# MIT-SPARK/TEASER-plusplus

Hardware: AMD Instinct MI355X
Metric: registrations/sec at N=10000 correspondences, 95% outliers (higher is better)
Workload: dtype bf16x3-split MFMA + f32 filter with FP64 fix-up for K1 (bitmap bit-identical to FP64); f64 estimators

## Files before the change

### teaser-plusplus_amd/csrc/kernels_graph.hip

```cpp
#include <algorithm>
#include <utility>
#include <vector>

#include <cstdio>
#include <cstdlib>

#include "internal.h"
#include "fixup_item.h"
#include "fixup_regions.h"
#include "k1_consts.h"
#include "wave_utils.h"

namespace thip {

struct EdgeConst {
  double beta;
  double beta2;
  double m2beta2;
  double beta4;
  double s_hat;
};

__device__ __forceinline__ bool tim_edge_exact(double ax, double ay, double az, double bx,
                                               double by, double bz, double beta) {
  const double A = (ax * ax + ay * ay) + az * az;
  const double B = (bx * bx + by * by) + bz * bz;
  return __builtin_fabs(__builtin_sqrt(A) - __builtin_sqrt(B)) <= beta;
}

__device__ __forceinline__ bool tim_edge_fast(double ax, double ay, double az, double bx,
                                              double by, double bz, const EdgeConst& k,
                                              bool* uncertain, bool* short_pair) {
  const double A = __builtin_fma(az, az, __builtin_fma(ay, ay, ax * ax));
  const double B = __builtin_fma(bz, bz, __builtin_fma(by, by, bx * bx));
  const double t = A + B;
  const double D = A - B;
  const double d = __builtin_fma(D, D, __builtin_fma(t, k.m2beta2, k.beta4));
  const double band = __builtin_fma(t, t, k.beta4) * 2e-12;
  *uncertain = !(__builtin_fabs(d) > band);
  *short_pair = t <= k.beta2;
  return d <= 0.0;
}

__device__ __forceinline__ bool tim_edge_scaled(double ax, double ay, double az, double bx,
                                                double by, double bz, const EdgeConst& k) {
  const double v1 = __builtin_sqrt((ax * ax + ay * ay) + az * az);
  const double v2 = __builtin_sqrt((bx * bx + by * by) + bz * bz);
  const double raw = v2 / v1;
  const double alpha = k.beta * (1.0 / v1);
  return __builtin_fabs(raw - k.s_hat) <= alpha;
}

constexpr int kColTilesPerWave = 4;
constexpr int kWavesPerBlock = 4;
constexpr int kColTilesPerBlock = kColTilesPerWave * kWavesPerBlock;

typedef double d2 __attribute__((ext_vector_type(2)));

template <int MODE>
struct ColTile {
  static constexpr int kPf = 3;
  const double* cb;
  d2 pf[kPf][3];
  int cb_addr;

  template <int C>
  __device__ __forceinline__ void load_col(d2 (&slot)[3]) {
    asm volatile("ds_read_b128 %0, %1 offset:%2" : "=v"(slot[0]) : "v"(cb_addr), "n"(48 * C));
    asm volatile("ds_read_b128 %0, %1 offset:%2" : "=v"(slot[1]) : "v"(cb_addr), "n"(48 * C + 16));
    asm volatile("ds_read_b128 %0, %1 offset:%2" : "=v"(slot[2]) : "v"(cb_addr), "n"(48 * C + 32));
  }
  double six, siy, siz, dix, diy, diz;
  unsigned int own_lo, own_hi;
  int tr_lo, tr_hi;
  uint64_t unc_cols;

  template <int B>
  __device__ __forceinline__ void step(const EdgeConst& kc) {
    constexpr int S = B % kPf;
    constexpr int younger = 3 * ((63 - B) < (kPf - 1) ? (63 - B) : (kPf - 1));
    asm volatile("s_waitcnt lgkmcnt(%3)" : "+v"(pf[S][0]), "+v"(pf[S][1]), "+v"(pf[S][2]) : "n"(younger));
    const double sjx = pf[S][0].x, sjy = pf[S][0].y, sjz = pf[S][1].x;
    const double djx = pf[S][1].y, djy = pf[S][2].x, djz = pf[S][2].y;
    if (B + kPf < 64) load_col<B + kPf>(pf[S]);
    bool e;
    uint64_t m;
    if (MODE == 0) {
      bool unc, shortp;
      const bool neg = tim_edge_fast(sjx - six, sjy - siy, sjz - siz, djx - dix, djy - diy,
                                     djz - diz, kc, &unc, &shortp);
      unc_cols |= (__builtin_amdgcn_ballot_w64(unc) != 0ull) ? (1ull << B) : 0ull;
      m = __builtin_amdgcn_ballot_w64(neg) | __builtin_amdgcn_ballot_w64(shortp);
// ... 211 lines not shown
  double H = 0.0;
  for (int k = 0; k < 6; ++k) {
    const float hi = f32_unkey(pr->hi[k]), lo = f32_unkey(~pr->lo[k]);
    const double e = 0.5 * ((double)hi - (double)lo);
    H = e > H ? e : H;
  }
  return H;
}

__global__ __launch_bounds__(256) void tim_prep_pack2_kernel(const ProbDesc* __restrict__ descs,
                                                             const double* __restrict__ src,
                                                             const double* __restrict__ dst,
                                                             TimPrep* __restrict__ prep,
                                                             TimOperandTile2* __restrict__ ops,
                                                             int32_t* __restrict__ deg, double beta) {
  const ProbDesc d = descs[blockIdx.y];
  const int ip = blockIdx.x * 256 + threadIdx.x;
  float mx = 0.f;
  if (ip < d.W * 64 && d.n > 0) {
    double g;
    int kexp;
    k1c::scale(beta, &g, &kexp);
    const int i = min(ip, d.n - 1);
    const TimPrep* pr = prep + blockIdx.y;
    const int sh = k1c::norm_shift(prep_half_extent(pr));
    kexp += 2 * sh;
    g *= k1c::pow2_d(sh);
    const double* a = src + 3 * (d.pt_off + i);
    const double* b = dst + 3 * (d.pt_off + i);
    const float sx = (float)((a[0] - prep_centre(pr, 0, 0)) * g), sy = (float)((a[1] - prep_centre(pr, 0, 1)) * g),
                sz = (float)((a[2] - prep_centre(pr, 0, 2)) * g);
    const float dx = (float)((b[0] - prep_centre(pr, 1, 0)) * g), dy = (float)((b[1] - prep_centre(pr, 1, 1)) * g),
                dz = (float)((b[2] - prep_centre(pr, 1, 2)) * g);
    const double na_d = ((double)sx * sx + (double)sy * sy) + (double)sz * sz;
    const double nb_d = ((double)dx * dx + (double)dy * dy) + (double)dz * dz;
    const float na = (float)na_d, nb = (float)nb_d;
    int ra, rb, pa, pb;
    k1c::xy_shifts(kexp, &ra, &rb, &pa, &pb);
    const float fra = (float)k1c::pow2_d(-ra), frb = (float)k1c::pow2_d(-rb), fpa = (float)k1c::pow2_d(-pa);
    const unsigned short P = f16_bits((float)k1c::pow2_d(-pb));
    unsigned short A[32], B[32];
    for (int k = 0; k < 32; ++k) A[k] = B[k] = 0;
    const float cs[3] = {sx, sy, sz}, cd[3] = {dx, dy, dz};
    float h, m, l;
    for (int c = 0; c < 3; ++c) {
      f16_split3(cs[c] * fra, &h, &m, &l);
      A[3 * c] = f16_bits(h); A[3 * c + 1] = A[3 * c]; A[3 * c + 2] = f16_bits(m);
      f16_split3(cs[c] * frb, &h, &m, &l);
      B[3 * c] = f16_bits(2.0f * h); B[3 * c + 1] = f16_bits(2.0f * m); B[3 * c + 2] = B[3 * c];
      f16_split3(cd[c] * fra, &h, &m, &l);
      A[16 + 3 * c] = f16_bits(h); A[16 + 3 * c + 1] = A[16 + 3 * c]; A[16 + 3 * c + 2] = f16_bits(m);
      f16_split3(cd[c] * frb, &h, &m, &l);
      B[16 + 3 * c] = f16_bits(-2.0f * h); B[16 + 3 * c + 1] = f16_bits(-2.0f * m); B[16 + 3 * c + 2] = B[16 + 3 * c];
    }
    f16_split3(na * fpa, &h, &m, &l);
    A[9] = f16_bits(-h); A[10] = f16_bits(-m); A[11] = f16_bits(-l); B[9] = P; B[10] = P; B[11] = P;
    B[12] = A[9]; B[13] = A[10]; B[14] = A[11]; A[12] = P; A[13] = P; A[14] = P;
    f16_split3(nb * fpa, &h, &m, &l);
    A[25] = f16_bits(h); A[26] = f16_bits(m); A[27] = f16_bits(l); B[25] = P; B[26] = P; B[27] = P;
    B[28] = A[25]; B[29] = A[26]; B[30] = A[27]; A[28] = P; A[29] = P; A[30] = P;
    A[31] = 0xb400;
    B[31] = 0x3c00;
    TimOperandTile2* tile = ops + d.w_off + (ip >> 6);
    const int gq = (ip >> 5) & 1, cc = ip & 31;
    for (int mf = 0; mf < kTimRowOperands; ++mf)
      for (int hh = 0; hh < 2; ++hh) {
        const unsigned short* pa = A + 16 * mf + 8 * hh;
        tile->a[gq][mf][hh][cc] = make_uint4(pa[0] | ((unsigned int)pa[1] << 16), pa[2] | ((unsigned int)pa[3] << 16),
                                             pa[4] | ((unsigned int)pa[5] << 16), pa[6] | ((unsigned int)pa[7] << 16));
        if (mf >= kTimColOperands) continue;
        const unsigned short* pb = B + 16 * mf + 8 * hh;
        tile->b[gq][mf][hh][cc] = make_uint4(pb[0] | ((unsigned int)pb[1] << 16), pb[2] | ((unsigned int)pb[3] << 16),
                                             pb[4] | ((unsigned int)pb[5] << 16), pb[6] | ((unsigned int)pb[7] << 16));
      }
    mx = na > nb ? na : nb;
    if (!(mx == mx)) mx = INFINITY;
    if (ip < d.n) deg[d.pt_off + ip] = 0;
  }
  for (int o = 32; o > 0; o >>= 1) {
    const float t = __shfl_xor(mx, o, 64);
    mx = t > mx ? t : mx;
  }
  if ((threadIdx.x & 63) == 0 && mx > 0.f) atomicMax(&prep[blockIdx.y].r2_bits, __float_as_uint(mx));
}

#ifdef TEASER_K1_LAB
struct TimOperandTile3 {
  uint4 a[2][3][2][32];
  uint4 b[2][2][2][32];
};
__global__ __launch_bounds__(256) void tim_prep_pack3_kernel(const ProbDesc* __restrict__ descs,
                                                             const double* __restrict__ src,
                                                             const double* __restrict__ dst,
                                                             TimPrep* __restrict__ prep,
                                                             TimOperandTile3* __restrict__ ops,
                                                             int32_t* __restrict__ deg, double beta) {
  const ProbDesc d = descs[blockIdx.y];
  const int ip = blockIdx.x * 256 + threadIdx.x;
  float mx = 0.f;
  if (ip < d.W * 64 && d.n > 0) {
    double g;
    int kexp;
    k1c::scale(beta, &g, &kexp);
    const int i = min(ip, d.n - 1);
    const TimPrep* pr = prep + blockIdx.y;
    const int sh = k1c::norm_shift(prep_half_extent(pr));
    kexp += 2 * sh;
    g *= k1c::pow2_d(sh);
    const double* a = src + 3 * (d.pt_off + i);
    const double* b = dst + 3 * (d.pt_off + i);
    const float sx = (float)((a[0] - prep_centre(pr, 0, 0)) * g), sy = (float)((a[1] - prep_centre(pr, 0, 1)) * g),
                sz = (float)((a[2] - prep_centre(pr, 0, 2)) * g);
    const float dx = (float)((b[0] - prep_centre(pr, 1, 0)) * g), dy = (float)((b[1] - prep_centre(pr, 1, 1)) * g),
                dz = (float)((b[2] - prep_centre(pr, 1, 2)) * g);
    const double na_d = ((double)sx * sx + (double)sy * sy) + (double)sz * sz;
    const double nb_d = ((double)dx * dx + (double)dy * dy) + (double)dz * dz;
    const float na = (float)na_d, nb = (float)nb_d;
    const double beta2s = k1c::pow2_d(kexp - 2);
    const float kappa = (float)k1c::pow2_d(kexp);
    const float delta_row = (float)(nb_d - na_d - beta2s);
    const float delta_col = (float)(nb_d - na_d);
    unsigned short A[48], B[32];
    for (int k = 0; k < 48; ++k) A[k] = 0;
    for (int k = 0; k < 32; ++k) B[k] = 0;
    const float cs[3] = {sx, sy, sz}, cd[3] = {dx, dy, dz};
    const unsigned short one = 0x3c00;
    float h, m, l;
    for (int c = 0; c < 3; ++c) {
      f16_split3(cs[c], &h, &m, &l);
      B[3 * c] = f16_bits(2.0f * h); B[3 * c + 1] = f16_bits(2.0f * m); B[3 * c + 2] = B[3 * c];
      A[3 * c] = f16_bits(h); A[3 * c + 1] = A[3 * c]; A[3 * c + 2] = f16_bits(m);
      A[32 + 3 * c] = f16_bits(kappa * h); A[32 + 3 * c + 1] = A[32 + 3 * c]; A[32 + 3 * c + 2] = f16_bits(kappa * m);
      f16_split3(cd[c], &h, &m, &l);
      B[16 + 3 * c] = f16_bits(-2.0f * h); B[16 + 3 * c + 1] = f16_bits(-2.0f * m); B[16 + 3 * c + 2] = B[16 + 3 * c];
      A[16 + 3 * c] = f16_bits(h); A[16 + 3 * c + 1] = A[16 + 3 * c]; A[16 + 3 * c + 2] = f16_bits(m);
    }
    f16_split3(na, &h, &m, &l);
    B[9] = f16_bits(-h); B[10] = f16_bits(-m);
    A[32 + 9] = f16_bits(kappa); A[32 + 10] = A[32 + 9];
    B[11] = one; B[12] = one; B[13] = one;
    B[14] = f16_bits(kappa); B[15] = B[14];
    A[32 + 14] = f16_bits(-h); A[32 + 15] = f16_bits(-m);
    f16_split3(delta_row, &h, &m, &l);
    A[11] = f16_bits(h); A[12] = f16_bits(m); A[13] = f16_bits(l);
    f16_split3(delta_col, &h, &m, &l);
    A[25] = one; A[26] = one; A[27] = one; B[25] = f16_bits(h); B[26] = f16_bits(m); B[27] = f16_bits(l);
    TimOperandTile3* tile = ops + d.w_off + (ip >> 6);
    const int gq = (ip >> 5) & 1, cc = ip & 31;
    for (int mf = 0; mf < 3; ++mf)
      for (int hh = 0; hh < 2; ++hh) {
        const unsigned short* pa = A + 16 * mf + 8 * hh;
        tile->a[gq][mf][hh][cc] = make_uint4(pa[0] | ((unsigned int)pa[1] << 16), pa[2] | ((unsigned int)pa[3] << 16),
                                             pa[4] | ((unsigned int)pa[5] << 16), pa[6] | ((unsigned int)pa[7] << 16));
        if (mf >= kTimColOperands) continue;
        const unsigned short* pb = B + 16 * mf + 8 * hh;
        tile->b[gq][mf][hh][cc] = make_uint4(pb[0] | ((unsigned int)pb[1] << 16), pb[2] | ((unsigned int)pb[3] << 16),
                                             pb[4] | ((unsigned int)pb[5] << 16), pb[6] | ((unsigned int)pb[7] << 16));
      }
    mx = na > nb ? na : nb;
    if (!(mx == mx)) mx = INFINITY;
    if (ip < d.n) deg[d.pt_off + ip] = 0;
  }
  for (int o = 32; o > 0; o >>= 1) {
    const float t = __shfl_xor(mx, o, 64);
    mx = t > mx ? t : mx;
  }
  if ((threadIdx.x & 63) == 0 && mx > 0.f) atomicMax(&prep[blockIdx.y].r2_bits, __float_as_uint(mx));
}
#endif

__global__ void tim_prep_consts_kernel(TimPrep* __restrict__ prep, int batch, double beta) {
  const int p = blockIdx.x * blockDim.x + threadIdx.x;
  if (p >= batch) return;
  const k1c::ConstsXY c = k1c::consts_xy(beta, k1c::norm_shift(prep_half_extent(prep + p)), prep[p].r2_bits);
  prep[p].band_c = c.C;
  prep[p].use_mfma = c.use_mfma;
}
#ifdef TEASER_K1_LAB
__global__ void tim_prep_consts3_kernel(TimPrep* __restrict__ prep, int batch, double beta) {
  const int p = blockIdx.x * blockDim.x + threadIdx.x;
  if (p >= batch) return;
  const k1c::Consts c = k1c::consts(beta, k1c::norm_shift(prep_half_extent(prep + p)), prep[p].r2_bits);
  prep[p].band_c = c.C;
  prep[p].use_mfma = c.use_mfma;
}
#endif


constexpr bool kK1Pipe = false, kK1Plain = true;
constexpr int kK1Chunks = 1, kK1Occ = 3;

template <bool PIPE, bool PLAIN, int OCC, int CHUNKS, bool LOWER, bool UW3 = false>
__global__ __launch_bounds__(256, OCC) void tim_graph_mfma3_kernel(
    const ProbDesc* __restrict__ descs, const double* __restrict__ src,
    const double* __restrict__ dst, const void* __restrict__ ops, const TimPrep* __restrict__ prep,
    uint64_t* __restrict__ bitmap, double beta, int gyr,
    unsigned long long* __restrict__ work, unsigned int* __restrict__ work_count,
    ProbState* __restrict__ states, int32_t* __restrict__ deg, unsigned long long* __restrict__ regions, int Tmax) {
  const ProbDesc d = descs[blockIdx.y];
  const int n = d.n, W = d.W;
  const int T = W;
  int Ig, X;
  fxr::decode_block((int)blockIdx.x, (int)gridDim.x, gyr, CHUNKS, &Ig, &X);
  constexpr int kBlockColTiles = kMfmaColTiles * CHUNKS;
  const int I0 = Ig * kMfmaRowTiles, Jbase = X * kBlockColTiles;
  auto region_of = [&](int wv, int chunk) -> unsigned long long* {
    const int Iw = I0 + wv, Xc = X * CHUNKS + chunk;
    return fxr::is_cell(Iw, Xc, Tmax) ? regions + fxr::region_offset((int)blockIdx.y, Tmax, Iw, Xc) : nullptr;
  };
  auto zero_regions = [&]() {
    if ((threadIdx.x & 63) < CHUNKS) {
      unsigned long long* r = region_of((int)(threadIdx.x >> 6), (int)(threadIdx.x & 63));
      if (r) r[0] = 0ull;
    }
  };
  if (I0 >= T || Jbase >= T || Jbase + kBlockColTiles - 1 < I0) {
    zero_regions();
    return;
  }
  const int lane = threadIdx.x & 63;
  const int wave = __builtin_amdgcn_readfirstlane(threadIdx.x >> 6);
  const int I = I0 + wave;

  const double* __restrict__ ps = src + 3 * d.pt_off;
  const double* __restrict__ pd = dst + 3 * d.pt_off;
  uint64_t* __restrict__ bm = bitmap + d.bm_off;
  __shared__ __attribute__((aligned(16))) uint64_t lds_own[kMfmaRowTiles][64][kMfmaColTiles + 1];
  static_assert(sizeof(lds_own[0]) >= sizeof(double) * 64 * 6 && sizeof(lds_own[0]) >= 8 * kWorkBuf, "aliased buffers");
  __shared__ __attribute__((aligned(16))) uint64_t lds_tr[kMfmaColTiles][64][kMfmaRowTiles];
  constexpr int kRowOps = UW3 ? 3 : kTimRowOperands;
  constexpr int kTileBytes = 2 * (kRowOps + kTimColOperands) * 1024, kColBase = 2 * kRowOps * 1024;
  static_assert(UW3 || (kTileBytes == (int)sizeof(TimOperandTile2) && kColBase == (int)offsetof(TimOperandTile2, b)), "tile layout");
  const char* __restrict__ qt = reinterpret_cast<const char*>(ops) + (size_t)d.w_off * kTileBytes;
  const int h = lane >> 5, c = lane & 31;
  typedef unsigned int u32x4 __attribute__((ext_vector_type(4)));
  const __amdgpu_buffer_rsrc_t q_rsrc = __builtin_amdgcn_make_buffer_rsrc(
      (void*)qt, 0, (int)((unsigned int)T * (unsigned int)kTileBytes), 0x00020000);
  auto load_op = [&](int tile, int side, int g, int m) -> uint4 {
    const int soff = tile * kTileBytes + (side ? kColBase + (g * kTimColOperands + m) * 1024 : (g * kRowOps + m) * 1024);
    const u32x4 v = __builtin_amdgcn_raw_buffer_load_b128(q_rsrc, lane * 16, soff, 0);
    return make_uint4(v.x, v.y, v.z, v.w);
  };
  f16x8 ar[2][kRowOps];
  {
    const int It = min(I, T - 1);
    for (int rt = 0; rt < 2; ++rt)
      for (int m = 0; m < kRowOps; ++m) ar[rt][m] = __builtin_bit_cast(f16x8, load_op(It, 0, rt, m));
  }
  const bool rowvalid = I < T;
  const uint64_t rowmask = !rowvalid ? 0ull : (n - I * 64 >= 64) ? ~0ull : ((1ull << (n - I * 64)) - 1ull);
  const int Jfirst = max(Jbase, I), Jend = min(Jbase + kBlockColTiles, T);
  uint4 bX[kTimColOperands], bY[kTimColOperands];
  {
    const int Jf = min(Jfirst, T - 1);
    for (int m = 0; m < kTimColOperands; ++m) bX[m] = load_op(Jf, 1, 0, m);
    if (PIPE)
      for (int m = 0; m < kTimColOperands; ++m) bY[m] = load_op(Jf, 1, 1, m);
  }
  const TimPrep pr = prep[blockIdx.y];
  if (!pr.use_mfma) {
// ... 419 lines not shown
      atomicAdd(dg + col, e ? 1 : -1);
    }
  };
  __shared__ unsigned long long queue[4][2 * kRegionWords];
  static_assert(kRegionWords == 64, "one region = one 64-lane load");
  const int T = W, nch = fxr::n_chunks(T);
  auto round = [&](int cnt, int tile) {
    if (lane < cnt) {
      const int col = min(fxi::col(queue[wave][lane]), n - 1);
      double* cp = col_pts[wave][lane];
      const double c0 = ps[3 * col], c1 = ps[3 * col + 1], c2 = ps[3 * col + 2];
      const double e0 = pd[3 * col], e1 = pd[3 * col + 1], e2 = pd[3 * col + 2];
      cp[0] = c0; cp[1] = c1; cp[2] = c2; cp[3] = e0; cp[4] = e1; cp[5] = e2;
    }
    __builtin_amdgcn_fence(__ATOMIC_ACQ_REL, "wavefront");
#pragma nounroll
    for (int base = 0; base < cnt; base += 4) {
      const int k = base + sub;
      resolve(queue[wave][k], k < cnt, std::true_type(), tile, k);
    }
    __builtin_amdgcn_fence(__ATOMIC_ACQ_REL, "wavefront");
  };
  const int wv = blockIdx.x * 4 + wave, nwv = gridDim.x * 4, npairs = (T + 1) >> 1;
  for (int pi = wv; pi < npairs; pi += nwv) {
    for (int side = 0; side < 2; ++side) {
      const int tile = side ? T - 1 - pi : pi;
      if (side && tile == pi) break;
      {
        const int pr = min(tile * 64 + lane, n - 1);
        double* rp = row_pts[wave][lane];
        rp[0] = ps[3 * pr]; rp[1] = ps[3 * pr + 1]; rp[2] = ps[3 * pr + 2];
        rp[3] = pd[3 * pr]; rp[4] = pd[3 * pr + 1]; rp[5] = pd[3 * pr + 2];
      }
      const int Xc0 = fxr::first_chunk(tile);
      const unsigned long long* reg = regions + fxr::region_offset(prob, Tmax, tile, Xc0);
      int qn = 0;
      unsigned long long mine = reg[lane];
      for (int Xc = Xc0; Xc < nch; ++Xc) {
        const unsigned long long cur = mine;
        if (Xc + 1 < nch) mine = reg[(size_t)(Xc + 1 - Xc0) * kRegionWords + lane];
        const int cnt = min((int)__builtin_amdgcn_readfirstlane((unsigned int)cur), kRegionItems);
        if (cnt <= 0) continue;
        if (lane >= 1 && lane <= cnt) queue[wave][qn + lane - 1] = cur;
        qn += cnt;
        if (qn >= kRegionWords) {
          __builtin_amdgcn_fence(__ATOMIC_ACQ_REL, "wavefront");
          round(kRegionWords, tile);
          qn -= kRegionWords;
          const unsigned long long moved = queue[wave][kRegionWords + lane];
          __builtin_amdgcn_fence(__ATOMIC_ACQ_REL, "wavefront");
          if (lane < qn) queue[wave][lane] = moved;
        }
      }
      if (qn > 0) {
        __builtin_amdgcn_fence(__ATOMIC_ACQ_REL, "wavefront");
        round(qn, tile);
      }
    }
  }
  const unsigned long long* seg = work + (((size_t)tpr.seg_off_hi << 32) | (size_t)tpr.seg_off_lo);
  const unsigned int ngrp = gridDim.x * 16;
  for (unsigned int w = (blockIdx.x * 256 + threadIdx.x) >> 4; w < total; w += ngrp) resolve(seg[w], true, std::false_type(), 0, 0);
}

constexpr int kMirrorRun = 8;
__global__ __launch_bounds__(256) void tim_mirror_lower_kernel(const ProbDesc* __restrict__ descs,
                                                               uint64_t* __restrict__ bitmap,
                                                               const ProbState* __restrict__ states, int skip_closed) {
  const ProbDesc d = descs[blockIdx.y];
  const int n = d.n, W = d.W, T = W;
  if (T < 2 || (skip_closed && states[blockIdx.y].deg_closed)) return;
  const int lane = threadIdx.x & 63;
  const int runs = (T + kMirrorRun - 1) / kMirrorRun;
  uint64_t* bm = bitmap + d.bm_off;
  for (int wv = blockIdx.x * 4 + (int)(threadIdx.x >> 6); wv < T * runs; wv += gridDim.x * 4) {
    const int J = wv / runs, Ia = (wv % runs) * kMirrorRun, Ib = min(Ia + kMirrorRun, J);
    if (Ia >= Ib) continue;
    uint64_t out[kMirrorRun];
#pragma unroll
    for (int k = 0; k < kMirrorRun; ++k) {
      out[k] = 0ull;
      if (Ia + k >= Ib) continue;
      const uint64_t x = bm[(int64_t)(64 * (Ia + k) + lane) * W + J];
#pragma unroll
      for (int c = 0; c < 64; ++c) {
        const uint64_t m = __builtin_amdgcn_ballot_w64(((x >> c) & 1ull) != 0ull);
        out[k] = lane == c ? m : out[k];
      }
    }
    const int row = 64 * J + lane;
    if (row < n) {
#pragma unroll
      for (int k = 0; k < kMirrorRun; ++k)
        if (Ia + k < Ib) bm[(int64_t)row * W + Ia + k] = out[k];
    }
  }
}

void launch_tim_graph(hipStream_t s, const ProbDesc* d_desc, int batch, int max_n,
                      const double* d_src, const double* d_dst, uint64_t* d_bitmap,
                      double noise_bound, double cbar2, int mode, const ProbState* d_state) {
  if (batch <= 0 || max_n <= 0) return;
  const int T = (max_n + 63) / 64;
  const double beta = 2 * noise_bound * sqrt(cbar2);
  const int gx = (T + kColTilesPerBlock - 1) / kColTilesPerBlock, gy = T;
  dim3 grid(gx * gy, batch);
  if (mode == 0)
    hipLaunchKernelGGL(tim_graph_kernel<0>, grid, dim3(256), 0, s, d_desc, d_src, d_dst, d_bitmap,
                       beta, gx, gy, d_state);
  else
    hipLaunchKernelGGL(tim_graph_kernel<1>, grid, dim3(256), 0, s, d_desc, d_src, d_dst, d_bitmap,
                       beta, gx, gy, d_state);
}

int64_t tim_prep_bytes(int batch) { return (int64_t)batch * ((int64_t)sizeof(TimPrep) + 4) + 64; }
#ifdef TEASER_K1_LAB
int64_t tim_operand_bytes(int64_t total_tiles) { return total_tiles * (int64_t)sizeof(TimOperandTile3); }
#else
int64_t tim_operand_bytes(int64_t total_tiles) { return total_tiles * (int64_t)sizeof(TimOperandTile2); }
#endif

static int tim_mfma_blocks(int T, int chunks) { return fxr::blocks(T, chunks); }
static int64_t tim_region_words(int max_n) { return fxr::arena_words((max_n + 63) / 64); }

static int64_t tim_segment_items(int n) {
  const int64_t seg = std::max<int64_t>((int64_t)n * (n - 1) / 2 / 256, 1 << 16);
  return std::min<int64_t>(seg, 0x7fffffffll);
}
int64_t tim_work_items(const int32_t* n, int batch) {
  int64_t segs = 0;
  int max_n = 0;
  for (int b = 0; b < batch; ++b) {
    segs += tim_segment_items(n[b]);
    max_n = std::max(max_n, n[b]);
  }
  return segs + tim_region_words(max_n) * std::max(batch, 1);
}
int64_t tim_prep_fill_segments(void* host_prep, const int32_t* n, int batch) {
  TimPrep* pr = reinterpret_cast<TimPrep*>(host_prep);
  int64_t off = 0;
  for (int b = 0; b < batch; ++b) {
    const int64_t seg = tim_segment_items(n[b]);
    pr[b].seg_off_lo = (unsigned int)((uint64_t)off & 0xffffffffu);
    pr[b].seg_off_hi = (unsigned int)((uint64_t)off >> 32);
    pr[b].seg_cap = (unsigned int)seg;
    off += seg;
  }
  return off;
}

int tim_probe_worklist(const void* d_prep, const void* d_work, int64_t work_cap, int batch, int max_n,
                       unsigned long long* regions_out, int64_t* stride_words, int64_t* used_regions,
                       unsigned int* seg_counts) {
  const int64_t reg_words = tim_region_words(max_n);
  *stride_words = reg_words;
  *used_regions = fxr::cells((max_n + 63) / 64);
  if (!regions_out) return 0;
  const unsigned long long* regions = reinterpret_cast<const unsigned long long*>(d_work) + (work_cap - reg_words * (int64_t)batch);
  hipError_t e = hipMemcpy(regions_out, regions, (size_t)reg_words * (size_t)batch * 8, hipMemcpyDeviceToHost);
  if (e == hipSuccess && seg_counts)
    e = hipMemcpy(seg_counts, reinterpret_cast<const char*>(d_prep) + sizeof(TimPrep) * (size_t)batch, 4 * (size_t)batch,
                  hipMemcpyDeviceToHost);
  return (int)e;
}

#ifdef TEASER_K1_LAB
struct K1Variant { int pipe, plain, chunks, occ4, uw3; };
static K1Variant k1_lab_variant() {
  const char* ev = getenv("TEASER_K1_VARIANT");
  const int v = ev ? atoi(ev) : 0;
  K1Variant k;
  k.uw3 = (v / 10000) % 10 != 0;
  k.occ4 = (v / 1000) % 10 != 0;
  k.pipe = v % 10 != 0;
  k.plain = (v / 10) % 10 != 0;
  k.chunks = 1 << ((v / 100) % 10);
  return k;
}
#endif

void launch_tim_graph_mfma(hipStream_t s, int phase, const ProbDesc* d_desc, int batch, int max_n,
                           int64_t total_tiles, const double* d_src, const double* d_dst,
                           void* d_pk, void* d_prep, void* d_work, int64_t work_cap,
                           uint64_t* d_bitmap, ProbState* d_state, int32_t* d_deg, double noise_bound,
                           double cbar2) {
  if (batch <= 0 || max_n <= 0) return;
  (void)total_tiles;
  const int T = (max_n + 63) / 64;
  if (phase == kTimMirror || phase == kTimMirrorOpen) {
    if (T < 2) return;
    const int waves = T * ((T + kMirrorRun - 1) / kMirrorRun);
    hipLaunchKernelGGL(tim_mirror_lower_kernel, dim3((unsigned)std::min(64, (waves + 3) / 4), batch), dim3(256), 0, s, d_desc,
                       d_bitmap, d_state, phase == kTimMirrorOpen ? 1 : 0);
    return;
  }
#ifdef TEASER_K1_LAB
  const bool upper = false;
#else
  const bool upper = (phase & kTimUpperOnly) != 0;
#endif
  phase &= ~kTimUpperOnly;
  const double beta = 2 * noise_bound * sqrt(cbar2);
  TimPrep* prep = reinterpret_cast<TimPrep*>(d_prep);
  unsigned long long* work = reinterpret_cast<unsigned long long*>(d_work);
  unsigned int* work_count = reinterpret_cast<unsigned int*>(reinterpret_cast<char*>(d_prep) +
                                                            sizeof(TimPrep) * (size_t)batch);
  const int64_t reg_words = tim_region_words(max_n);
  unsigned long long* regions = work + (work_cap - reg_words * (int64_t)batch);
#ifdef TEASER_K1_LAB
  const K1Variant lab = k1_lab_variant();
#endif
  if (phase == 0) {
    hipLaunchKernelGGL(tim_prep_bbox_kernel, dim3((max_n + 1023) / 1024, batch), dim3(256), 0, s, d_desc,
                       d_src, d_dst, prep);
#ifdef TEASER_K1_LAB
    if (lab.uw3) {
      hipLaunchKernelGGL(tim_prep_pack3_kernel, dim3((T * 64 + 255) / 256, batch), dim3(256), 0, s, d_desc, d_src,
                         d_dst, prep, reinterpret_cast<TimOperandTile3*>(d_pk), d_deg, beta);
      hipLaunchKernelGGL(tim_prep_consts3_kernel, dim3((batch + 63) / 64), dim3(64), 0, s, prep, batch, beta);
      return;
    }
#endif
    hipLaunchKernelGGL(tim_prep_pack2_kernel, dim3((T * 64 + 255) / 256, batch), dim3(256), 0, s, d_desc, d_src,
                       d_dst, prep, reinterpret_cast<TimOperandTile2*>(d_pk), d_deg, beta);
    hipLaunchKernelGGL(tim_prep_consts_kernel, dim3((batch + 63) / 64), dim3(64), 0, s, prep, batch, beta);
  } else if (phase == 1) {
    const int gyr = (T + kMfmaRowTiles - 1) / kMfmaRowTiles;
#define TIM_K1_LAUNCH(PIPE, PLAIN, CHUNKS) TIM_K1_LAUNCH_OCC(PIPE, PLAIN, kK1Occ, CHUNKS, true)
#define TIM_K1_LAUNCH_OCC(PIPE, PLAIN, OCC, CHUNKS, ...)                                                                       \
  hipLaunchKernelGGL((tim_graph_mfma3_kernel<PIPE, PLAIN, OCC, CHUNKS, __VA_ARGS__>), dim3(tim_mfma_blocks(T, CHUNKS), batch), \
                     dim3(256), 0, s, d_desc, d_src, d_dst, (const void*)d_pk, prep, d_bitmap, beta, gyr, work, work_count,    \
                     d_state, d_deg, regions, T)
#ifdef TEASER_K1_LAB
#define TIM_K1_LAB_CASE(PIPE, PLAIN)                             \
  if (lab.pipe == (PIPE ? 1 : 0) && lab.plain == (PLAIN ? 1 : 0)) { \
    if (lab.chunks == 1) { TIM_K1_LAUNCH(PIPE, PLAIN, 1); }      \
    else if (lab.chunks == 2) { TIM_K1_LAUNCH(PIPE, PLAIN, 2); } \
    else { TIM_K1_LAUNCH(PIPE, PLAIN, 4); }                      \
  }
    if (lab.uw3) {
      if (lab.plain) { TIM_K1_LAUNCH_OCC(false, true, kK1Occ, 1, true, true); } else { TIM_K1_LAUNCH_OCC(false, false, kK1Occ, 1, true, true); }
    } else if (lab.occ4) {
      if (lab.plain) { TIM_K1_LAUNCH_OCC(false, true, 4, 1, true); } else { TIM_K1_LAUNCH_OCC(false, false, 4, 1, true); }
    } else {
      TIM_K1_LAB_CASE(false, false)
      TIM_K1_LAB_CASE(false, true)
      TIM_K1_LAB_CASE(true, false)
      TIM_K1_LAB_CASE(true, true)
    }
#undef TIM_K1_LAB_CASE
#else
    if (upper) {
      TIM_K1_LAUNCH_OCC(kK1Pipe, kK1Plain, kK1Occ, kK1Chunks, false);
    } else {
      TIM_K1_LAUNCH(kK1Pipe, kK1Plain, kK1Chunks);
    }
#endif
#undef TIM_K1_LAUNCH
#undef TIM_K1_LAUNCH_OCC
  } else {
    const int64_t forced_wgs = setting(S_FIXUP_WGS);
    const int64_t fix_wgs = forced_wgs > 0 ? forced_wgs : ((T + 1) / 2 + 3) / 4;
    hipLaunchKernelGGL(tim_fixup_group_kernel, dim3((unsigned)std::max<int64_t>(4, fix_wgs), batch),
                       dim3(256), 0, s, d_desc, batch, d_src, d_dst, d_bitmap, beta, work, work_count, d_state, d_deg,
                       regions, T, prep, upper ? 1 : 0);
  }
}

__global__ __launch_bounds__(256) void degree_kernel(const ProbDesc* __restrict__ descs,
                                                     const uint64_t* __restrict__ bitmap,
                                                     int32_t* __restrict__ deg) {
  const ProbDesc d = descs[blockIdx.y];
  const int lane = threadIdx.x & 63;
  for (int row = blockIdx.x * 4 + (threadIdx.x >> 6); row < d.n; row += gridDim.x * 4) {
    const uint64_t* r = bitmap + d.bm_off + (int64_t)row * d.W;
    int c = 0;
    for (int w = lane; w < d.W; w += 64) c += __popcll(r[w]);
    c = wave_sum_i(c);
    if (lane == 0) deg[d.pt_off + row] = c;
  }
}

void launch_degrees(hipStream_t s, const ProbDesc* d_desc, int batch, int max_n,
                    const uint64_t* d_bitmap, int32_t* d_deg, ProbState* d_state) {
  if (batch <= 0 || max_n <= 0) return;
  dim3 grid((max_n + 3) / 4, batch);
  hipLaunchKernelGGL(degree_kernel, grid, dim3(256), 0, s, d_desc, d_bitmap, d_deg);
}

__global__ __launch_bounds__(256) void trims_kernel(const double* __restrict__ src,
                                                    const double* __restrict__ dst, int n,
                                                    double beta, double* __restrict__ raw,
                                                    double* __restrict__ alpha) {
  const int i = blockIdx.x;
  if (i >= n - 1) return;
  const int64_t seg = (int64_t)i * n - (int64_t)i * (i + 1) / 2;
  const double six = src[3 * i], siy = src[3 * i + 1], siz = src[3 * i + 2];
  const double dix = dst[3 * i], diy = dst[3 * i + 1], diz = dst[3 * i + 2];
  for (int j = i + 1 + threadIdx.x; j < n; j += 256) {
    const double ax = src[3 * j] - six, ay = src[3 * j + 1] - siy, az = src[3 * j + 2] - siz;
    const double bx = dst[3 * j] - dix, by = dst[3 * j + 1] - diy, bz = dst[3 * j + 2] - diz;
    const double v1 = __builtin_sqrt((ax * ax + ay * ay) + az * az);
    const double v2 = __builtin_sqrt((bx * bx + by * by) + bz * bz);
    const int64_t k = seg + (j - i - 1);
    raw[k] = v2 / v1;
    alpha[k] = beta * (1.0 / v1);
  }
}
// ... 33 lines not shown
```

### teaser-plusplus_amd/csrc/kernels_heuristic.hip

```cpp
#include <algorithm>
#include <utility>
#include <vector>

#include <cstdio>
#include <cstdlib>

#include "internal.h"
#include "wave_utils.h"

namespace thip {

constexpr int kGreedyMaxThreads = 512;
constexpr int kCap = 640;
constexpr int kCapW = kCap / 64;
constexpr int kCapStride = kCapW + 1;

template <int kGreedyWaves>
__device__ __forceinline__ int blockN_sum_i(int v, int* red ) {
  v = wave_sum_i(v);
  __syncthreads();
  if ((threadIdx.x & 63) == 0) red[threadIdx.x >> 6] = v;
  __syncthreads();
  int s = 0;
#pragma unroll
  for (int k = 0; k < kGreedyWaves; ++k) s += red[k];
  return s;
}
template <int kGreedyWaves>
__device__ __forceinline__ unsigned long long blockN_max_u64(unsigned long long v,
                                                             unsigned long long* red) {
  v = wave_max_u64(v);
  __syncthreads();
  if ((threadIdx.x & 63) == 0) red[threadIdx.x >> 6] = v;
  __syncthreads();
  unsigned long long m = 0;
#pragma unroll
  for (int k = 0; k < kGreedyWaves; ++k) m = red[k] > m ? red[k] : m;
  return m;
}

template <int kGreedyThreads>
__device__ __forceinline__ int greedy_one_start(
    const ProbDesc* __restrict__ descs, const uint64_t* __restrict__ bitmap,
    const int32_t* __restrict__ deg, ProbState* __restrict__ states,
    int32_t* __restrict__ start_cliques, int64_t total_n, char* smem, const int sidx, long long* trace, const int prob) {
  constexpr int kGreedyWaves = kGreedyThreads / 64;
  long long* tr = trace ? trace + ((size_t)prob * kMaxStarts + sidx) * 8 : nullptr;
  auto stamp = [&](int k) {
    if (tr && threadIdx.x == 0) tr[k] = (long long)wall_clock64();
  };
  auto bump = [&](int k) {
    if (tr && threadIdx.x == 0) tr[k] += 1;
  };
  if (tr && threadIdx.x == 0) tr[6] = tr[7] = 0;
  stamp(0);
  const ProbDesc d = descs[prob];
  const int n = d.n, W = d.W;
  const int Wpad = (W + 1) & ~1;
  uint64_t* P = reinterpret_cast<uint64_t*>(smem);
  uint64_t* U = P + Wpad;
  uint64_t* A = U + Wpad;
  uint64_t* Pc = A + kCap * kCapStride;
  unsigned long long* red64 = reinterpret_cast<unsigned long long*>(Pc + 16);
  int* cand = reinterpret_cast<int*>(red64 + kGreedyMaxThreads / 64);
  int* wcnt = cand + kCap;
  int* red = wcnt + kGreedyMaxThreads;
  int* misc = red + kGreedyMaxThreads / 64;

  ProbState* st = states + prob;
  const int tid = threadIdx.x, lane = tid & 63, wave = tid >> 6;
  const uint64_t* bm = bitmap + d.bm_off;
  const int32_t* dg = deg + d.pt_off;
  int32_t* C = start_cliques + (int64_t)sidx * total_n + d.pt_off;
  int v0 = -1;
  {
    unsigned long long best = 0, sum = 0;
    for (int v = sidx + kMaxStarts * tid; v < n; v += kMaxStarts * kGreedyThreads) {
      const unsigned long long dv = (unsigned int)dg[v];
      const unsigned long long key = ((dv + 1) << 32) | (0xffffffffu - (unsigned int)v);
      best = key > best ? key : best;
    }
    best = blockN_max_u64<kGreedyWaves>(best, red64);
    if (best) v0 = (int)(0xffffffffu - (unsigned int)(best & 0xffffffffu));
    if (sidx == 0) {
      for (int v = tid; v < n; v += kGreedyThreads) sum += (unsigned int)dg[v];
#pragma unroll
      for (int o = 32; o > 0; o >>= 1) sum += __shfl_xor(sum, o, 64);
      __syncthreads();
      if (lane == 0) red64[wave] = sum;
      __syncthreads();
      if (tid == 0) {
// ... 726 lines not shown
#pragma unroll
        for (int r = 0; r < kRows; ++r)
#pragma unroll
          for (int u = 0; u < kRowStageWords / 64; ++u)
            if (64 * u < W) rowbuf[wave][r][64 * u + lane] = wv[r][u];
        __builtin_amdgcn_fence(__ATOMIC_ACQ_REL, "wavefront");
      }
      const unsigned int* rowlds = reinterpret_cast<const unsigned int*>(&rowbuf[wave][0][0]);
      auto groups = [&](auto staged_tag) {
        constexpr bool STAGED = decltype(staged_tag)::value;
        for (int g0 = 0; g0 < ng; g0 += kGrp) {
          unsigned int x[kRows][kGrp];
          int cbit[kGrp], cdeg[kGrp];
#pragma unroll
          for (int q = 0; q < kGrp; ++q) {
            const int idx = 64 * (g0 + q) + lane;
            const unsigned int key = idx < m ? keys[idx] : 0u;
            const int c = (int)(key & 0xffffu);
            cdeg[q] = idx < m ? (int)(key >> 16) : -1;
            cbit[q] = c & 31;
#pragma unroll
            for (int r = 0; r < kRows; ++r)
              x[r][q] = (cdeg[q] >= 0 && (c >> 6) >= rtile[r]) ? (STAGED ? rowlds[r * 2 * kRowStageWords + (c >> 5)] : rp[r][c >> 5]) : 0u;
          }
#pragma unroll
          for (int q = 0; q < kGrp; ++q) {
            if (g0 + q >= ng) break;
#pragma unroll
            for (int r = 0; r < kRows; ++r) {
              const uint64_t mask = __ballot(((x[r][q] >> cbit[q]) & 1u) != 0u);
              if (lane == g0 + q) myword[r] = mask;
            }
          }
        }
      };
      if (staged)
        groups(std::true_type());
      else
        groups(std::false_type());
#pragma unroll
      for (int r = 0; r < kRows; ++r)
        if (rb + r < k1 && lane < kCoreWords) comp[(size_t)(rb + r) * kCoreWords + lane] = myword[r];
      __builtin_amdgcn_fence(__ATOMIC_ACQ_REL, "wavefront");
    }
  }
}

__global__ __launch_bounds__(kDegThreads) void degree_closure_symmetrise_kernel(
    const uint64_t* __restrict__ part_pool ,
    uint64_t* __restrict__ comp_pool ,
    int32_t* __restrict__ h_pool , const uint32_t* __restrict__ key_pool ,
    const int32_t* __restrict__ counters, int batch) {
  TAIL_WAVE_PRIO();
  __shared__ unsigned short cdeg[kCoreCap];
  constexpr int kOutWords = 8;
  __shared__ uint64_t outbuf[kDegThreads / 64][64][kOutWords + 1];
  static_assert(kCoreCap <= 65535 && kDegBins >= kCoreCap, "clamped degrees fit and stay ordered");
  const int m = counters[blockIdx.y];
  if (m < 2) return;
  const int tid = threadIdx.x, lane = tid & 63, wave = tid >> 6;
  {
    const uint32_t* kin = key_pool + (size_t)blockIdx.y * kCoreCap;
    for (int r = tid; r < m; r += kDegThreads) cdeg[r] = (unsigned short)min(kin[r] >> 16, (uint32_t)kCoreCap);
  }
  __syncthreads();
  const int ng = (m + 63) >> 6;
  const uint64_t* part = part_pool + (size_t)blockIdx.y * kCoreCap * kCoreWords;
  uint64_t* comp = comp_pool + (size_t)blockIdx.y * kCoreCap * kCoreWords;
  int32_t* hout = h_pool + (size_t)blockIdx.y * kCoreCap;
  for (int A = blockIdx.x * 4 + wave; A < ng; A += gridDim.x * 4) {
    const int row = 64 * A + lane;
    const bool rowok = row < m;
    int base = 0, hmax = 0;
    uint64_t own_n = rowok ? part[(size_t)row * kCoreWords] : 0ull;
    uint64_t src_n = lane < m ? part[(size_t)lane * kCoreWords + A] : 0ull;
    for (int B = 0; B < ng; ++B) {
      const uint64_t own = own_n, src = src_n;
      if (B + 1 < ng) {
        const int trow = 64 * (B + 1) + lane;
        own_n = rowok ? part[(size_t)row * kCoreWords + B + 1] : 0ull;
        src_n = trow < m ? part[(size_t)trow * kCoreWords + A] : 0ull;
      }
      uint64_t tr = 0ull;
      if (__builtin_amdgcn_ballot_w64(src != 0ull) != 0ull) {
#pragma unroll
        for (int c = 0; c < 64; ++c) {
          const uint64_t mk = __builtin_amdgcn_ballot_w64(((src >> c) & 1ull) != 0ull);
          tr = lane == c ? mk : tr;
        }
      }
      const uint64_t full = rowok ? (own | tr) : 0ull;
      outbuf[wave][lane][B & (kOutWords - 1)] = full;
      const int cnt = __popcll(full);
      const int cols = min(64, m - 64 * B);
      const int d_hi = cdeg[64 * B], d_lo = cdeg[64 * B + cols - 1];
      const bool below = base + cnt <= d_lo;
      const bool above = base + 1 >= d_hi;
      if (__builtin_amdgcn_ballot_w64(cnt > 0 && !below && !above) != 0ull) {
        for (int k = 0; k < cols; ++k) {
          const uint64_t upto = k == 63 ? ~0ull : ((2ull << k) - 1ull);
          const int P = base + __popcll(full & upto);
          const int cand = min(P, (int)cdeg[64 * B + k]);
          hmax = ((full >> k) & 1ull) ? max(hmax, cand) : hmax;
        }
      } else if (cnt > 0) {
        hmax = max(hmax, below ? base + cnt : (int)cdeg[64 * B + __builtin_ctzll(full)]);
      }
      base += cnt;
      if ((B & (kOutWords - 1)) == kOutWords - 1 || B == ng - 1) {
        __builtin_amdgcn_fence(__ATOMIC_ACQ_REL, "wavefront");
        const int w = lane & (kOutWords - 1), Bw = (B & ~(kOutWords - 1)) + w;
#pragma unroll
        for (int it = 0; it < 8; ++it) {
          const int r = it * 8 + (lane >> 3);
          if (64 * A + r < m && Bw <= B) comp[(size_t)(64 * A + r) * kCoreWords + Bw] = outbuf[wave][r][w];
        }
        __builtin_amdgcn_fence(__ATOMIC_ACQ_REL, "wavefront");
      }
    }
    if (rowok) hout[row] = hmax;
  }
}

constexpr int kCoverMax = 4;
constexpr int kMissCap = 64;
__global__ __launch_bounds__(kDegThreads) void degree_closure_verdict_kernel(
    const ProbDesc* __restrict__ descs, ProbState* __restrict__ states, int32_t* __restrict__ clique,
    const uint64_t* __restrict__ comp_pool, const int32_t* __restrict__ h_pool, const uint32_t* __restrict__ key_pool,
    const int32_t* __restrict__ counters, int batch) {
  TAIL_WAVE_PRIO();
  __shared__ uint64_t Pa[kDegMaxW];
  __shared__ int hist[kCoreCap + 1];
  __shared__ int hval[kCoreCap];
  __shared__ uint64_t Sa[kCoreWords], Sb[kCoreWords];
  __shared__ int csum[kDegThreads];
  __shared__ unsigned long long red64[4];
  __shared__ int miss_n, miss_verdict;
  __shared__ unsigned short miss_a[kMissCap], miss_b[kMissCap];
  const int m = counters[blockIdx.x], t = counters[batch + blockIdx.x];
  if (m < 2) return;
  const ProbDesc d = descs[blockIdx.x];
  ProbState* st = states + blockIdx.x;
  const int W = d.W, tid = threadIdx.x, lane = tid & 63, wave = tid >> 6;
  const int ng = (m + 63) >> 6;
  const uint64_t* comp = comp_pool + (size_t)blockIdx.x * kCoreCap * kCoreWords;
  const int32_t* hout = h_pool + (size_t)blockIdx.x * kCoreCap;
  const uint32_t* keys = key_pool + (size_t)blockIdx.x * kCoreCap;
  constexpr int kHBins = kCoreCap;
  for (int i = tid; i <= kHBins; i += kDegThreads) hist[i] = 0;
  __syncthreads();
  for (int r = tid; r < m; r += kDegThreads) {
    const int hv = hout[r];
    hval[r] = hv;
    atomicAdd(&hist[hv < kHBins ? hv : kHBins], 1);
  }
  __syncthreads();
  suffix_counts<kHBins>(hist, csum, tid);
  constexpr int kPerH = kHBins / kDegThreads;
  int kmax = kHBins;
  for (int attempt = 0; attempt < 8; ++attempt) {
    int kb = 0;
    {
      int c = csum[tid];
#pragma unroll
      for (int k = kPerH - 1; k >= 0; --k) {
        const int j = tid * kPerH + k;
        c += hist[j];
        if (c >= j + 1 && j + 1 <= kmax && j + 1 > kb) kb = j + 1;
      }
    }
    const int k = (int)block_max_u64((unsigned long long)kb, red64);
    if (k < 2 || k - 1 < t) return;
    __syncthreads();
// ... 800 lines not shown
```

Baseline: 110,200.

## Replace ballot-loop 64x64 bit transpose with permlane/DPP butterfly and fuse consts kernel

Adds a shared 64x64 bit-matrix transpose that uses permlane32/16 swaps, DPP lane shuffles and bitop3 masking. It replaces the 64-iteration ballot-and-select loops in the lower-triangle mirror kernel and in the heuristic core transpose. This cuts each transpose from 64 ballots to a handful of cross-lane steps. Separately, the per-problem constants computation moves into the pack kernel: the last block to finish, found with an atomic ticket counter, computes the constants, which removes one kernel launch. The ticket scheme relies on pad[0] being zero before the first launch and on correct fence ordering, and the new intrinsics need gfx950-class hardware.

Result: no change. 112,100 (median of 3 runs) (+1.7%).

```diff
diff --git a/teaser-plusplus_amd/csrc/bit_transpose.h b/teaser-plusplus_amd/csrc/bit_transpose.h
--- /dev/null
+++ b/teaser-plusplus_amd/csrc/bit_transpose.h
@@ -0,0 +1,60 @@
+#pragma once
+#include <cstdint>
+
+namespace bt {
+
+constexpr uint64_t kKeepMask[6] = {0x00000000FFFFFFFFull, 0x0000FFFF0000FFFFull, 0x00FF00FF00FF00FFull,
+                                   0x0F0F0F0F0F0F0F0Full, 0x3333333333333333ull, 0x5555555555555555ull};
+
+#if defined(__HIPCC__)
+__device__ __forceinline__ uint64_t transpose64(uint64_t x, int lane) {
+  const auto r32 = __builtin_amdgcn_permlane32_swap((unsigned int)x, (unsigned int)(x >> 32), false, false);
+  unsigned int h[2] = {r32[0], r32[1]};
+  const unsigned int sel16 = (lane & 16) ? 0x03020706u : 0x01000504u;
+#pragma unroll
+  for (int hf = 0; hf < 2; ++hf) {
+    unsigned int y;
+    {
+      const auto sw = __builtin_amdgcn_permlane16_swap(h[hf], h[hf], false, false);
+      y = __builtin_amdgcn_perm(sw[0], sw[1], sel16);
+    }
+#pragma unroll
+    for (int st = 2; st < 6; ++st) {
+      const int j = 32 >> st;
+      unsigned int p;
+      switch (st) {
+        case 2: p = __builtin_amdgcn_update_dpp(0u, y, 0x128, 0xf, 0xf, true); break;
+        case 3:
+          p = __builtin_amdgcn_update_dpp(0u, y, 0x141, 0xf, 0xf, true);
+          p = __builtin_amdgcn_update_dpp(0u, p, 0x1b, 0xf, 0xf, true);
+          break;
+        case 4: p = __builtin_amdgcn_update_dpp(0u, y, 0x4e, 0xf, 0xf, true); break;
+        default: p = __builtin_amdgcn_update_dpp(0u, y, 0xb1, 0xf, 0xf, true); break;
+      }
+      const bool up = (lane & j) != 0;
+      const unsigned int shifted = __builtin_amdgcn_alignbit(p, p, up ? j : 32 - j);
+      const unsigned int km = (unsigned int)kKeepMask[st];
+      y = __builtin_amdgcn_bitop3_b32(up ? ~km : km, y, shifted, 0xCA);
+    }
+    h[hf] = y;
+  }
+  return ((uint64_t)h[1] << 32) | h[0];
+}
+#endif
+
+#ifndef __HIP_DEVICE_COMPILE__
+inline void host_transpose64(uint64_t x[64]) {
+  for (int st = 0; st < 6; ++st) {
+    const int j = 32 >> st;
+    const uint64_t m = kKeepMask[st];
+    uint64_t y[64];
+    for (int l = 0; l < 64; ++l) {
+      const uint64_t p = x[l ^ j];
+      y[l] = (l & j) ? ((x[l] & ~m) | ((p >> j) & m)) : ((x[l] & m) | ((p << j) & ~m));
+    }
+    for (int l = 0; l < 64; ++l) x[l] = y[l];
+  }
+}
+#endif
+
+}
diff --git a/teaser-plusplus_amd/csrc/kernels_graph.hip b/teaser-plusplus_amd/csrc/kernels_graph.hip
--- a/teaser-plusplus_amd/csrc/kernels_graph.hip
+++ b/teaser-plusplus_amd/csrc/kernels_graph.hip
@@ -8,6 +8,7 @@
 #include "internal.h"
 #include "fixup_item.h"
 #include "fixup_regions.h"
+#include "bit_transpose.h"
 #include "k1_consts.h"
 #include "wave_utils.h"
 
@@ -385,6 +386,20 @@
     mx = t > mx ? t : mx;
   }
   if ((threadIdx.x & 63) == 0 && mx > 0.f) atomicMax(&prep[blockIdx.y].r2_bits, __float_as_uint(mx));
+  asm volatile("s_waitcnt vmcnt(0)" ::: "memory");
+  __syncthreads();
+  if (threadIdx.x == 0) {
+    TimPrep* pr = prep + blockIdx.y;
+    const unsigned int ticket = __hip_atomic_fetch_add(&pr->pad[0], 1u, __ATOMIC_RELAXED, __HIP_MEMORY_SCOPE_AGENT);
+    if (ticket == gridDim.x - 1) {
+      __builtin_amdgcn_fence(__ATOMIC_ACQUIRE, "agent");
+      const unsigned int r2 = atomicMax(&pr->r2_bits, 0u);
+      const k1c::ConstsXY c = k1c::consts_xy(beta, k1c::norm_shift(prep_half_extent(pr)), r2);
+      pr->band_c = c.C;
+      pr->use_mfma = c.use_mfma;
+      __hip_atomic_store(&pr->pad[0], 0u, __ATOMIC_RELAXED, __HIP_MEMORY_SCOPE_AGENT);
+    }
+  }
 }
 
 #ifdef TEASER_K1_LAB
@@ -472,13 +487,6 @@
 }
 #endif
 
-__global__ void tim_prep_consts_kernel(TimPrep* __restrict__ prep, int batch, double beta) {
-  const int p = blockIdx.x * blockDim.x + threadIdx.x;
-  if (p >= batch) return;
-  const k1c::ConstsXY c = k1c::consts_xy(beta, k1c::norm_shift(prep_half_extent(prep + p)), prep[p].r2_bits);
-  prep[p].band_c = c.C;
-  prep[p].use_mfma = c.use_mfma;
-}
 #ifdef TEASER_K1_LAB
 __global__ void tim_prep_consts3_kernel(TimPrep* __restrict__ prep, int batch, double beta) {
   const int p = blockIdx.x * blockDim.x + threadIdx.x;
@@ -1064,11 +1072,7 @@
       out[k] = 0ull;
       if (Ia + k >= Ib) continue;
       const uint64_t x = bm[(int64_t)(64 * (Ia + k) + lane) * W + J];
-#pragma unroll
-      for (int c = 0; c < 64; ++c) {
-        const uint64_t m = __builtin_amdgcn_ballot_w64(((x >> c) & 1ull) != 0ull);
-        out[k] = lane == c ? m : out[k];
-      }
+      out[k] = bt::transpose64(x, lane);
     }
     const int row = 64 * J + lane;
     if (row < n) {
@@ -1205,7 +1209,6 @@
 #endif
     hipLaunchKernelGGL(tim_prep_pack2_kernel, dim3((T * 64 + 255) / 256, batch), dim3(256), 0, s, d_desc, d_src,
                        d_dst, prep, reinterpret_cast<TimOperandTile2*>(d_pk), d_deg, beta);
-    hipLaunchKernelGGL(tim_prep_consts_kernel, dim3((batch + 63) / 64), dim3(64), 0, s, prep, batch, beta);
   } else if (phase == 1) {
     const int gyr = (T + kMfmaRowTiles - 1) / kMfmaRowTiles;
 #define TIM_K1_LAUNCH(PIPE, PLAIN, CHUNKS) TIM_K1_LAUNCH_OCC(PIPE, PLAIN, kK1Occ, CHUNKS, true)
diff --git a/teaser-plusplus_amd/csrc/kernels_heuristic.hip b/teaser-plusplus_amd/csrc/kernels_heuristic.hip
--- a/teaser-plusplus_amd/csrc/kernels_heuristic.hip
+++ b/teaser-plusplus_amd/csrc/kernels_heuristic.hip
@@ -7,6 +7,7 @@
 
 #include "internal.h"
 #include "wave_utils.h"
+#include "bit_transpose.h"
 
 namespace thip {
 
@@ -899,13 +900,7 @@
         src_n = trow < m ? part[(size_t)trow * kCoreWords + A] : 0ull;
       }
       uint64_t tr = 0ull;
-      if (__builtin_amdgcn_ballot_w64(src != 0ull) != 0ull) {
-#pragma unroll
-        for (int c = 0; c < 64; ++c) {
-          const uint64_t mk = __builtin_amdgcn_ballot_w64(((src >> c) & 1ull) != 0ull);
-          tr = lane == c ? mk : tr;
-        }
-      }
+      if (__builtin_amdgcn_ballot_w64(src != 0ull) != 0ull) tr = bt::transpose64(src, lane);
       const uint64_t full = rowok ? (own | tr) : 0ull;
       outbuf[wave][lane][B & (kOutWords - 1)] = full;
       const int cnt = __popcll(full);
```
